# dropbox/divans

Hardware: AMD Instinct MI355X
Metric: MB/s encode+decode per GPU, 64 KiB metablocks; bit-exact vs CPU (higher is better)
Workload: dtype u16/u64 integer

## Files before the change

### divans_amd/csrc/lit_bucket.hip

```cpp
#include "lit_bucket_dev.h"

namespace divans_hip {

__global__ __launch_bounds__(BK_SORT_THREADS) void bucket_sort_kernel(const BucketBatch b) {
    __shared__ __attribute__((aligned(16))) uint8_t staging[BK_PIECE];
    __shared__ __attribute__((aligned(16))) uint8_t piece_in[16 + BK_PIECE];
    __shared__ uint32_t hist[4][256];
    __shared__ uint32_t scan[256];
    const uint32_t s = blockIdx.x / b.pieces, piece = blockIdx.x % b.pieces;
    const uint32_t tid = threadIdx.x, w = tid >> 6, lane = tid & 63;
    const uint32_t len = b.in_sizes ? b.in_sizes[s] : b.stream_len;
    const uint8_t* in = b.in + (b.in_offsets ? b.in_offsets[s] : (uint64_t)s * b.stream_len);
    uint32_t* desc = b.desc + ((size_t)s * 256u + tid) * 8u + piece;
    const uint32_t base = piece * BK_PIECE;
    if (base >= len) { *desc = 0u; return; }
    const uint32_t n = len - base < BK_PIECE ? len - base : BK_PIECE;
    const size_t pl = b.slot;
    for (uint32_t i = tid; i < 1024u; i += BK_SORT_THREADS) (&hist[0][0])[i] = 0u;
    {
        const uint8_t* src = in + base;
        if ((((uintptr_t)src) & 15u) == 0u) {
            for (uint32_t i = tid * 16u; i < n; i += BK_SORT_THREADS * 16u) {
                if (i + 16u <= n) *(u32x4*)(piece_in + 16u + i) = *(const u32x4*)(src + i);
                else for (uint32_t k = i; k < n; ++k) piece_in[16u + k] = src[k];
            }
        } else {
            for (uint32_t i = tid; i < n; i += BK_SORT_THREADS) piece_in[16u + i] = src[i];
        }
        if (tid == 0u) piece_in[15] = base ? in[base - 1u] : 0u;
    }
    __syncthreads();
    const uint8_t* key_of = piece_in + 15;
    for (uint32_t bt = 0; bt < 32u; ++bt) {
        const uint32_t p = w * 2048u + bt * 64u + lane;
        if (p < n) atomicAdd(&hist[w][key_of[p]], 1u);
    }
    __syncthreads();
    const uint32_t c0 = hist[0][tid], c1 = hist[1][tid], c2 = hist[2][tid], c3 = hist[3][tid];
    const uint32_t tot = c0 + c1 + c2 + c3;
    scan[tid] = tot;
    __syncthreads();
    for (uint32_t d = 1; d < 256u; d <<= 1) {
        const uint32_t v = tid >= d ? scan[tid - d] : 0u;
        __syncthreads();
        scan[tid] += v;
        __syncthreads();
    }
    const uint32_t start = scan[tid] - tot;
    hist[0][tid] = start; hist[1][tid] = start + c0; hist[2][tid] = start + c0 + c1; hist[3][tid] = start + c0 + c1 + c2;
    *desc = start | (tot << 16);
    __syncthreads();
    uint16_t* inv = b.inv + (size_t)s * pl + base;
    for (uint32_t bt = 0; bt < 32u; ++bt) {
        const uint32_t p = w * 2048u + bt * 64u + lane;
        const bool valid = p < n;
        const uint32_t key = valid ? key_of[p] : 0u;
        const uint32_t byte = valid ? key_of[p + 1u] : 0u;
        unsigned long long same = __ballot(valid);
        for (uint32_t bit = 0; bit < 8u; ++bit) {
            const bool set = (key >> bit) & 1u;
            const unsigned long long bb = __ballot(set);
            same &= set ? bb : ~bb;
        }
        const uint32_t rank = lanes_below(same), cnt = (uint32_t)__popcll(same);
        if (valid) {
            const uint32_t off = hist[w][key];
            staging[off + rank] = (uint8_t)byte;
            inv[p] = (uint16_t)(off + rank);
            if (rank == cnt - 1u) hist[w][key] = off + cnt;
        }
    }
    __syncthreads();
    uint8_t* sorted = b.sorted + (size_t)s * pl + base;
    for (uint32_t i = tid * 16u; i < n; i += BK_SORT_THREADS * 16u) {
        if (i + 16u <= n) *(u32x4*)(sorted + i) = *(const u32x4*)(staging + i);
        else for (uint32_t k = i; k < n; ++k) sorted[k] = staging[k];
    }
}

__global__ __launch_bounds__(1024) void bucket_tasks_kernel(const BucketBatch b) {
    __shared__ uint32_t cnt[BK_CLASSES], basev[BK_CLASSES];
    const uint32_t t = blockIdx.x * 1024u + threadIdx.x;
    const uint32_t cap = b.n_streams * 256u;
    if (threadIdx.x < BK_CLASSES) cnt[threadIdx.x] = 0u;
    __syncthreads();
    uint32_t tot = 0;
    if (t < cap) {
        const u32x4* d = (const u32x4*)(b.desc + (size_t)t * 8u);
        const u32x4 d0 = d[0], d1 = d[1];
        tot = (d0.x >> 16) + (d0.y >> 16) + (d0.z >> 16) + (d0.w >> 16) + (d1.x >> 16) + (d1.y >> 16) + (d1.z >> 16) + (d1.w >> 16);
    }
    const int cls = bk_class_of(tot);
    uint32_t local = 0;
    for (int c = 0; c < (int)BK_CLASSES; ++c) {
        const unsigned long long m = __ballot(cls == c);
        if (m == 0ull) continue;
        const int leader = __ffsll((long long)m) - 1;
        uint32_t wbase = 0;
        if ((int)(threadIdx.x & 63u) == leader) wbase = atomicAdd(&cnt[c], (uint32_t)__popcll(m));
        wbase = (uint32_t)__builtin_amdgcn_readlane((int)wbase, leader);
        if (cls == c) local = wbase + lanes_below(m);
    }
    __syncthreads();
    if (threadIdx.x < BK_CLASSES) basev[threadIdx.x] = cnt[threadIdx.x] ? atomicAdd(&b.counters[threadIdx.x], cnt[threadIdx.x]) : 0u;
    __syncthreads();
    if (cls >= 0) b.tasks[(size_t)cls * cap + basev[cls] + local] = t;
}

__global__ __launch_bounds__(64) void bucket_chain_kernel(const BucketBatch b) {
    extern __shared__ __attribute__((aligned(16))) uint32_t lds32[];
    const uint32_t lane = threadIdx.x;
    uint32_t* my = lds32 + lane * BK_LANE_DWORDS;
    uint32_t* mydesc = my + BK_DESC_DW;
    uint32_t* tab = lds32 + BK_TAB_DW;
    const uint32_t inc = (uint32_t)b.inc; const int lim = b.lim;
    for (uint32_t i = lane; i < 128u; i += 64u) {
        tab[i] = bk_tab_entry(i, inc);
    }
    __syncthreads();
    const size_t pl = b.slot;
    const uint32_t cap = b.n_streams * 256u;
    BkTaskLists lists; lists.load(b.counters);
    const uint32_t total = lists.total();
    const u32x4 def0 = {4u | (8u << 16), 12u | (16u << 16), 20u | (24u << 16), 28u | (32u << 16)};
    const u32x4 def1 = {36u | (40u << 16), 44u | (48u << 16), 52u | (56u << 16), 60u | (64u << 16)};

    bool has_task = false, exhausted = false;
    uint32_t run_i = 0, nruns = 0, left = 0, idx = 0;
    u32x2* cur_sfs = b.sfs; const uint8_t* cur_sorted = b.sorted;
    uint32_t nt_stage = 0, nt_tid = 0;
    u32x4 nd0 = {0u, 0u, 0u, 0u}, nd1 = {0u, 0u, 0u, 0u};
    uint32_t win_cur = 0, win_end = 0, nxt_val = 0, nxt_w = 0;
    const uint32_t long_end = lists.ends[3];
    bool nxt_pending = false, drained = false;
    u32x2 e_next = {0u, 0u}; uint32_t m_next = 0;
    u32x2 pv0 = {0u, 0u}, pv1 = pv0, pv2 = pv0, pv3 = pv0, pv4 = pv0, pv5 = pv0, pv6 = pv0, pv7 = pv0;
    uint32_t m_prev = 0; u32x2* sfs_prev = b.sfs;

#define BK_OPAQUE(X) asm volatile("" : "+v"(X))
#define BK_BYTE(K, WORD, PV)                                                                            \
    if (((K - first) & 15u) < cnt) {                                                                    \
        const uint32_t byte_ = (WORD >> (8u * (K & 3u))) & 0xffu;                                       \
        const uint32_t hi = byte_ >> 4, lo = byte_ & 15u;                                               \
        uint32_t* rowl = my + 8u * (1u + hi);                                                           \
        BkRow H = bk_read(my, tab, hi), L = bk_read(rowl, tab, lo);                                     \
        const u32x2 v = {bk_pack(H, hi), bk_pack(L, lo)};                                               \
        bk_add(H); bk_add(L);                                                                           \
        bk_renorm_at(H, lim); bk_renorm_at(L, lim);                                                     \
        *(u32x4*)my = H.w0; *(u32x4*)(my + 4) = H.w1; *(u32x4*)rowl = L.w0; *(u32x4*)(rowl + 4) = L.w1; \
        PV = v;                                                                                         \
    }

    for (;;) {
        u32x2 e = e_next; const uint32_t m = m_next;
        if (m_prev & BK_VALID) {
            u32x2* dst = sfs_prev + (m_prev & 0xffffu);
            const uint32_t pf = (m_prev >> 16) & 15u, pc = (m_prev >> 20) & 15u;
            if (pc == 8u) {
                const u32x4 q0 = {pv0.x, pv0.y, pv1.x, pv1.y}, q1 = {pv2.x, pv2.y, pv3.x, pv3.y};
                const u32x4 q2 = {pv4.x, pv4.y, pv5.x, pv5.y}, q3 = {pv6.x, pv6.y, pv7.x, pv7.y};
                bk_store_quad((u32x4*)dst, q0); bk_store_quad((u32x4*)(dst + 2), q1);
                bk_store_quad((u32x4*)(dst + 4), q2); bk_store_quad((u32x4*)(dst + 6), q3);
            } else {
                if (((0u - pf) & 15u) < pc) bk_store_pair(dst + 0, pv0);
                if (((1u - pf) & 15u) < pc) bk_store_pair(dst + 1, pv1);
                if (((2u - pf) & 15u) < pc) bk_store_pair(dst + 2, pv2);
                if (((3u - pf) & 15u) < pc) bk_store_pair(dst + 3, pv3);
                if (((4u - pf) & 15u) < pc) bk_store_pair(dst + 4, pv4);
                if (((5u - pf) & 15u) < pc) bk_store_pair(dst + 5, pv5);
                if (((6u - pf) & 15u) < pc) bk_store_pair(dst + 6, pv6);
                if (((7u - pf) & 15u) < pc) bk_store_pair(dst + 7, pv7);
            }
        }
        {
            const bool adv = has_task && left == 0u, more = run_i < nruns;
            const uint32_t d = mydesc[run_i & 7u];
            if (adv && more) { left = d >> 16; idx = d & 0xffffu; ++run_i; }
            if (adv && !more) has_task = false;
        }
        {
            const bool fetch_ = has_task && left != 0u;
            const uint32_t base = idx & ~7u, first_ = idx & 7u;
            const uint32_t cnt_ = left < 8u - first_ ? left : 8u - first_;
            const uint8_t* lp = fetch_ ? cur_sorted + base : b.sorted;
            e_next = *(const u32x2*)lp;
            m_next = fetch_ ? (base | (first_ << 16) | (cnt_ << 20) | BK_VALID) : 0u;
            idx += fetch_ ? cnt_ : 0u; left -= fetch_ ? cnt_ : 0u;
        }
        BK_OPAQUE(e);
        m_prev = m; sfs_prev = cur_sfs;
        if (m & BK_VALID) {
            const uint32_t first = (m >> 16) & 15u, cnt = (m >> 20) & 15u;
            BK_BYTE(0u, e.x, pv0) BK_BYTE(1u, e.x, pv1) BK_BYTE(2u, e.x, pv2) BK_BYTE(3u, e.x, pv3)
            BK_BYTE(4u, e.y, pv4) BK_BYTE(5u, e.y, pv5) BK_BYTE(6u, e.y, pv6) BK_BYTE(7u, e.y, pv7)
        }
        if (!has_task && !(m_next & BK_VALID) && nt_stage == 3u) {
            BK_OPAQUE(nd0); BK_OPAQUE(nd1);
            uint32_t n = 0;
            const uint32_t dsc[8] = {nd0.x, nd0.y, nd0.z, nd0.w, nd1.x, nd1.y, nd1.z, nd1.w};
#pragma unroll
            for (uint32_t j = 0; j < 8u; ++j) if (dsc[j] >> 16) { mydesc[n] = dsc[j] + j * BK_PIECE; ++n; }
            nruns = n; run_i = 0u;
            for (uint32_t r = 0; r < 17u; ++r) { *(u32x4*)(my + 8u * r) = def0; *(u32x4*)(my + 8u * r + 4u) = def1; }
            cur_sfs = b.sfs + (size_t)(nt_tid >> 8) * pl; cur_sorted = b.sorted + (size_t)(nt_tid >> 8) * pl;
            left = 0u; has_task = true; nt_stage = 0u;
        }
        const bool want = nt_stage == 0u && !exhausted;
        if (nt_stage == 2u) nt_stage = 3u;
        else if (nt_stage == 1u) {
            BK_OPAQUE(nt_tid);
            const u32x4* dp = (const u32x4*)(b.desc + (size_t)nt_tid * 8u);
            nd0 = dp[0]; nd1 = dp[1];
            nt_stage = 2u;
        }
        const unsigned long long wm = __ballot(want);
        if (wm) {
            if (win_cur == win_end && nxt_pending) {
                BK_OPAQUE(nxt_val);
                const uint32_t basev = (uint32_t)__builtin_amdgcn_readfirstlane((int)nxt_val);
                nxt_pending = false;
                if (basev >= total) { drained = true; win_cur = win_end = total; }
                else { win_cur = basev; win_end = basev + nxt_w < total ? basev + nxt_w : total; }
            }
            const uint32_t avail = win_end - win_cur, asked = (uint32_t)__popcll(wm);
            const uint32_t rank = lanes_below(wm);
            if (want) {
                if (rank < avail) {
                    const uint32_t t = win_cur + rank;
                    nt_tid = *lists.at(b.tasks, cap, t);
                    nt_stage = 1u;
                } else if (drained) exhausted = true;
            }
            win_cur += asked < avail ? asked : avail;
        }
        const uint32_t want_w = win_end < long_end ? 64u : BK_WINDOW;
        if (!nxt_pending && !drained && win_end - win_cur < want_w / 2u) {
            nxt_w = want_w;
            if (lane == 0u) nxt_val = atomicAdd(&b.counters[BK_CLAIM], want_w);
            nxt_pending = true;
        }
        const bool done = !has_task && !(m_next & BK_VALID) && !(m_prev & BK_VALID) && nt_stage == 0u && exhausted;
        if (__ballot(!done) == 0ull) break;
    }
#undef BK_BYTE
#undef BK_OPAQUE
}

__global__ __launch_bounds__(1024) void bucket_unsort_kernel(const BucketBatch b) {
    __shared__ u32x2 buf[BK_PIECE];
    const uint32_t s = blockIdx.x / b.pieces, piece = blockIdx.x % b.pieces;
    const uint32_t len = b.in_sizes ? b.in_sizes[s] : b.stream_len;
    const uint32_t base = piece * BK_PIECE;
    if (base >= len) return;
    const uint32_t n = len - base < BK_PIECE ? len - base : BK_PIECE;
    const size_t pl = b.slot;
    const u32x2* src = b.sfs + (size_t)s * pl + base;
    for (uint32_t i = threadIdx.x; i < n; i += 1024u) buf[i] = __builtin_nontemporal_load(src + i);
    __syncthreads();
    const uint16_t* inv = b.inv + (size_t)s * pl + base;
    u32x2* dst = (u32x2*)(b.sf + (size_t)s * b.sf_stride) + base;
    for (uint32_t i = threadIdx.x; i < n; i += 1024u) dst[i] = buf[inv[i]];
}

__global__ __launch_bounds__(1024) void bucket_unsort32_kernel(const BucketBatch b) {
    __shared__ uint32_t buf[BK_PIECE];
    const uint32_t s = blockIdx.x / b.pieces, piece = blockIdx.x % b.pieces;
    const uint32_t len = b.in_sizes ? b.in_sizes[s] : b.stream_len;
    const uint32_t base = piece * BK_PIECE;
    if (base >= len) return;
    const uint32_t n = len - base < BK_PIECE ? len - base : BK_PIECE;
    const size_t pl = b.slot;
    const uint32_t* src = (const uint32_t*)b.sfs + (size_t)s * pl + base;
    const uint32_t n2 = (n + 1u) & ~1u;
    for (uint32_t i = 2u * threadIdx.x; i < n2; i += 2048u) *(u32x2*)(buf + i) = __builtin_nontemporal_load((const u32x2*)(src + i));
    __syncthreads();
    const uint16_t* inv = b.inv + (size_t)s * pl + base;
    uint32_t* dst = b.sf + (size_t)s * b.sf_stride + base;
    for (uint32_t i = 2u * threadIdx.x; i < n2; i += 2048u) {
        const uint32_t iv = *(const uint32_t*)(inv + i);
        const u32x2 v = {buf[iv & 0xffffu], i + 1u < n ? buf[iv >> 16] : 0u};
        *(u32x2*)(dst + i) = v;
    }
}

uint32_t bucket_chain_lds_bytes() { return (64u * BK_LANE_DWORDS + 128u) * 4u; }

void launch_bucket_tasks(const BucketBatch& b, hipStream_t st) {
    hipLaunchKernelGGL(bucket_tasks_kernel, dim3((b.n_streams + 3u) / 4u), dim3(1024), 0, st, b);
}
void launch_bucket_unsort(const BucketBatch& b, hipStream_t st) {
    hipLaunchKernelGGL(bucket_unsort_kernel, dim3(b.n_streams * b.pieces), dim3(1024), 0, st, b);
}

void launch_bucket_unsort32(const BucketBatch& b, hipStream_t st) {
    hipLaunchKernelGGL(bucket_unsort32_kernel, dim3(b.n_streams * b.pieces), dim3(1024), 0, st, b);
}

hipError_t launch_bucket_model(const BucketBatch& b, uint32_t chain_blocks, hipStream_t st) {
    hipError_t e = hipMemsetAsync(b.counters, 0, 64, st);
    if (e != hipSuccess) return e;
    if (b.pieces < 8u) {
        e = hipMemsetAsync(b.desc, 0, (size_t)b.n_streams * 256u * 8u * sizeof(uint32_t), st);
        if (e != hipSuccess) return e;
    }
    hipLaunchKernelGGL(bucket_sort_kernel, dim3(b.n_streams * b.pieces), dim3(BK_SORT_THREADS), 0, st, b);
    hipLaunchKernelGGL(bucket_tasks_kernel, dim3((b.n_streams + 3u) / 4u), dim3(1024), 0, st, b);
    hipLaunchKernelGGL(bucket_chain_kernel, dim3(chain_blocks), dim3(64), bucket_chain_lds_bytes(), st, b);
    hipLaunchKernelGGL(bucket_unsort_kernel, dim3(b.n_streams * b.pieces), dim3(1024), 0, st, b);
    return hipGetLastError();
}

}
```

Baseline: 15070.

## Fuse histogram with in-wave ranking via LDS match masks and shuffle scan

The bucket sort kernel now computes each element's within-wave rank and per-wave bucket histogram in a single pass. It uses LDS atomic-or match masks instead of a separate atomicAdd histogram followed by an 8-ballot key-matching loop, and keeps the ranks in registers (kept[16]) for the scatter pass. The 256-entry block scan, which used many __syncthreads, is replaced by a wave shuffle scan plus a 4-entry cross-wave sum. A compile-time probe flag that disables chain-kernel stores is also added but is off by default. The cost is higher register pressure from the kept array and correctness that relies on LDS atomic ordering within a wave.

```diff
diff --git a/divans_amd/csrc/lit_bucket.hip b/divans_amd/csrc/lit_bucket.hip
--- a/divans_amd/csrc/lit_bucket.hip
+++ b/divans_amd/csrc/lit_bucket.hip
@@ -1,14 +1,19 @@
 #include "lit_bucket_dev.h"
 
+#ifndef DIVANS_BK_CHAIN_NO_STORES
+#define DIVANS_BK_CHAIN_NO_STORES 0
+#endif
+
 namespace divans_hip {
 
 __global__ __launch_bounds__(BK_SORT_THREADS) void bucket_sort_kernel(const BucketBatch b) {
-    __shared__ __attribute__((aligned(16))) uint8_t staging[BK_PIECE];
+    __shared__ __attribute__((aligned(16))) unsigned long long staging64[BK_PIECE / 8u];
+    uint8_t* staging = (uint8_t*)staging64;
     __shared__ __attribute__((aligned(16))) uint8_t piece_in[16 + BK_PIECE];
     __shared__ uint32_t hist[4][256];
-    __shared__ uint32_t scan[256];
+    __shared__ uint32_t wsum[4];
     const uint32_t s = blockIdx.x / b.pieces, piece = blockIdx.x % b.pieces;
-    const uint32_t tid = threadIdx.x, w = tid >> 6, lane = tid & 63;
+    const uint32_t tid = threadIdx.x, w = (uint32_t)__builtin_amdgcn_readfirstlane((int)(tid >> 6)), lane = tid & 63;
     const uint32_t len = b.in_sizes ? b.in_sizes[s] : b.stream_len;
     const uint8_t* in = b.in + (b.in_offsets ? b.in_offsets[s] : (uint64_t)s * b.stream_len);
     uint32_t* desc = b.desc + ((size_t)s * 256u + tid) * 8u + piece;
@@ -31,43 +36,49 @@
     }
     __syncthreads();
     const uint8_t* key_of = piece_in + 15;
+    unsigned long long* mask_of = staging64 + w * 256u;
+    const unsigned long long my_bit = 1ull << lane;
+    uint32_t kept[16];
+#pragma unroll
+    for (uint32_t bt = 0; bt < 32u; ++bt) {
+        uint32_t r = 0;
+        const uint32_t p = w * 2048u + bt * 64u + lane;
+        if (p < n) {
+            const uint32_t key = key_of[p];
+            __hip_atomic_store(mask_of + key, 0ull, __ATOMIC_RELAXED, __HIP_MEMORY_SCOPE_WORKGROUP);
+            __hip_atomic_fetch_or(mask_of + key, my_bit, __ATOMIC_RELAXED, __HIP_MEMORY_SCOPE_WORKGROUP);
+            const unsigned long long same = __hip_atomic_load(mask_of + key, __ATOMIC_RELAXED, __HIP_MEMORY_SCOPE_WORKGROUP);
+            const uint32_t rank = lanes_below(same), cnt = (uint32_t)__popcll(same);
+            const uint32_t before = hist[w][key];
+            r = before + rank;
+            if (rank == cnt - 1u) hist[w][key] = before + cnt;
+        }
+        if (bt & 1u) kept[bt >> 1] |= r << 16; else kept[bt >> 1] = r;
+    }
+    __syncthreads();
+    const uint32_t c0 = hist[0][tid], c1 = hist[1][tid], c2 = hist[2][tid], c3 = hist[3][tid];
+    const uint32_t tot = c0 + c1 + c2 + c3;
+    uint32_t incl = tot;
+    for (uint32_t d = 1; d < 64u; d <<= 1) {
+        const uint32_t v = (uint32_t)__shfl_up((int)incl, d, 64);
+        if (lane >= d) incl += v;
+    }
+    if (lane == 63u) wsum[w] = incl;
+    __syncthreads();
+    uint32_t start = incl - tot;
+    for (uint32_t j = 0; j < 3u; ++j) if (j < w) start += wsum[j];
+    hist[0][tid] = start; hist[1][tid] = start + c0; hist[2][tid] = start + c0 + c1; hist[3][tid] = start + c0 + c1 + c2;
+    *desc = start | (tot << 16);
+    __syncthreads();
+    uint16_t* inv = b.inv + (size_t)s * pl + base;
+#pragma unroll
     for (uint32_t bt = 0; bt < 32u; ++bt) {
         const uint32_t p = w * 2048u + bt * 64u + lane;
-        if (p < n) atomicAdd(&hist[w][key_of[p]], 1u);
-    }
-    __syncthreads();
-    const uint32_t c0 = hist[0][tid], c1 = hist[1][tid], c2 = hist[2][tid], c3 = hist[3][tid];
-    const uint32_t tot = c0 + c1 + c2 + c3;
-    scan[tid] = tot;
-    __syncthreads();
-    for (uint32_t d = 1; d < 256u; d <<= 1) {
-        const uint32_t v = tid >= d ? scan[tid - d] : 0u;
-        __syncthreads();
-        scan[tid] += v;
-        __syncthreads();
-    }
-    const uint32_t start = scan[tid] - tot;
-    hist[0][tid] = start; hist[1][tid] = start + c0; hist[2][tid] = start + c0 + c1; hist[3][tid] = start + c0 + c1 + c2;
-    *desc = start | (tot << 16);
-    __syncthreads();
-    uint16_t* inv = b.inv + (size_t)s * pl + base;
-    for (uint32_t bt = 0; bt < 32u; ++bt) {
-        const uint32_t p = w * 2048u + bt * 64u + lane;
-        const bool valid = p < n;
-        const uint32_t key = valid ? key_of[p] : 0u;
-        const uint32_t byte = valid ? key_of[p + 1u] : 0u;
-        unsigned long long same = __ballot(valid);
-        for (uint32_t bit = 0; bit < 8u; ++bit) {
-            const bool set = (key >> bit) & 1u;
-            const unsigned long long bb = __ballot(set);
-            same &= set ? bb : ~bb;
-        }
-        const uint32_t rank = lanes_below(same), cnt = (uint32_t)__popcll(same);
-        if (valid) {
-            const uint32_t off = hist[w][key];
-            staging[off + rank] = (uint8_t)byte;
-            inv[p] = (uint16_t)(off + rank);
-            if (rank == cnt - 1u) hist[w][key] = off + cnt;
+        if (p < n) {
+            const uint32_t key = key_of[p], byte = key_of[p + 1u];
+            const uint32_t slot = hist[w][key] + ((kept[bt >> 1] >> (16u * (bt & 1u))) & 0xffffu);
+            staging[slot] = (uint8_t)byte;
+            inv[p] = (uint16_t)slot;
         }
     }
     __syncthreads();
@@ -153,7 +164,12 @@
 
     for (;;) {
         u32x2 e = e_next; const uint32_t m = m_next;
+#if DIVANS_BK_CHAIN_NO_STORES
+        asm volatile("" : : "v"(pv0), "v"(pv1), "v"(pv2), "v"(pv3), "v"(pv4), "v"(pv5), "v"(pv6), "v"(pv7), "v"(sfs_prev));
+        if (false) {
+#else
         if (m_prev & BK_VALID) {
+#endif
             u32x2* dst = sfs_prev + (m_prev & 0xffffu);
             const uint32_t pf = (m_prev >> 16) & 15u, pc = (m_prev >> 20) & 15u;
             if (pc == 8u) {
@@ -305,6 +321,10 @@
     }
     hipLaunchKernelGGL(bucket_sort_kernel, dim3(b.n_streams * b.pieces), dim3(BK_SORT_THREADS), 0, st, b);
     hipLaunchKernelGGL(bucket_tasks_kernel, dim3((b.n_streams + 3u) / 4u), dim3(1024), 0, st, b);
+#if DIVANS_BK_CHAIN_NO_STORES
+    e = hipMemsetD32Async((hipDeviceptr_t)b.sfs, (int)(1u | (2048u << 16)), (size_t)b.n_streams * b.slot * 2u, st);
+    if (e != hipSuccess) return e;
+#endif
     hipLaunchKernelGGL(bucket_chain_kernel, dim3(chain_blocks), dim3(64), bucket_chain_lds_bytes(), st, b);
     hipLaunchKernelGGL(bucket_unsort_kernel, dim3(b.n_streams * b.pieces), dim3(1024), 0, st, b);
     return hipGetLastError();
```

After: 15290 (median of 6 runs). 1.01x the previous value.
